# pollen-robotics/reachy2_symbolic_ik

Hardware: AMD Instinct MI355X
Metric: IK solves/sec (7-DoF r_arm, batched poses) (higher is better)
Workload: dtype f64; 1 GPU; config2: r_arm is_reachable + theta_to_joints_func(interval[0]), 1048576 random reachable poses per GPU; poses_per_gpu=1048576, theta_policy=interval[0], collective=none

## Files before the change

reachy2_symbolic_ik_amd/csrc/rsik_device.hpp:

```cpp
#pragma once

#include <hip/hip_runtime.h>
#include <stdint.h>

#include "../../include/rsik.h"
#include "rsik_math.hpp"

namespace rsik {

#ifdef RSIK_HOT_ONLY
#define RSIK_RARE(c) (false)
#else
#define RSIK_RARE(c) (__builtin_expect(!!(c), 0))
#endif


#ifdef RSIK_ISA_MARKS
#define RSIK_MARK(name) asm volatile("; RSIK_MARK " name)
#else
#define RSIK_MARK(name)
#endif

constexpr double kPi = 3.141592653589793;
constexpr double kTwoPi = 2 * kPi;
// ... 150 lines not shown
    else if (fabs(mid - kPi) <= 1e-7) { first = -2 * half_diff; third = 0.0; }
    else { first = half_sum - half_diff; third = half_sum + half_diff; }
    mid -= kPi / 2;
    eul[0] = first; eul[1] = mid; eul[2] = third;
#pragma unroll
    for (int k = 0; k < 3; k++) {
        if (eul[k] < -kPi) eul[k] += kTwoPi;
        else if (eul[k] > kPi) eul[k] -= kTwoPi;
    }
}

struct Frame {
    V3 c0, c1, c2;
};
__device__ __forceinline__ bool frame_is_special(V3 u) {
    if (!RSIK_RARE(fmax(fabs(u.y), fabs(u.z)) < 2e-8)) return false;
    return np_isclose(0.0, u.y) && np_isclose(0.0, u.z);
}
__device__ __forceinline__ V3 frame_c0(V3 u) {
    V3 c0 = u;
    if (RSIK_RARE(frame_is_special(u))) {
        if (np_isclose(1.0, u.x)) c0 = {1, 0, 0};
        else if (np_isclose(1.0, -u.x)) c0 = {-1, 0, 0};
    }
    return c0;
}
__device__ __forceinline__ Frame frame_from_unit(V3 u, double h) {
    Frame F;
    double yh = u.y * h, zh = u.z * h;
    double yzh = u.y * zh;
    F.c0 = u;
    F.c1 = {-u.y, fma(-u.y, yh, 1.0), -yzh};
    F.c2 = {-u.z, -yzh, fma(-u.z, zh, 1.0)};
    if (RSIK_RARE(frame_is_special(u))) {
        if (np_isclose(1.0, u.x)) { F.c0 = {1, 0, 0}; F.c1 = {0, 1, 0}; F.c2 = {0, 0, 1}; }
        else if (np_isclose(1.0, -u.x)) { F.c0 = {-1, 0, 0}; F.c1 = {0, 1, 0}; F.c2 = {0, 0, -1}; }
    }
    return F;
}
__device__ __forceinline__ Frame frame_from_unit(V3 u) { return frame_from_unit(u, fast_rcp(1.0 + u.x)); }

struct Reach {
    int state;
    bool ok;
    double i0, i1;
    double ct0, st0;
    double ct1, st1;
    V3 pos;
    V3 w;
    V3 c2;
    double r2;
    V3 n2;
    V3 a1, a2;
    int stage;
};

template <class Acc>
__device__ __forceinline__ V3 cvec(const Acc& A, int off) {
    return {A(off), A(off + 1), A(off + 2)};
}

struct Goal {
    V3 woff, toff, xg;
    V3 tw;
};
template <class Acc>
__device__ __forceinline__ Goal make_goal(const Acc& A, const Rot& Rg) {
    const V3 tl = cvec(A, RSIK_C_TIPL);
    Goal g;
    g.woff = {Rg.m[0] * tl.x + Rg.m[1] * tl.y + Rg.m[2] * tl.z, Rg.m[3] * tl.x + Rg.m[4] * tl.y + Rg.m[5] * tl.z,
              Rg.m[6] * tl.x + Rg.m[7] * tl.y + Rg.m[8] * tl.z};
    g.toff = {fma(Rg.m[0], tl.x, Rg.m[1] * tl.y), fma(Rg.m[3], tl.x, Rg.m[4] * tl.y), fma(Rg.m[6], tl.x, Rg.m[7] * tl.y)};
    g.xg = Rg.col0();
    g.tw = {-(Rg.m[2] * tl.z), -(Rg.m[5] * tl.z), -(Rg.m[8] * tl.z)};
    return g;
}
template <class Acc>
__device__ __forceinline__ Goal goal_from_euler_tipz(const Acc& A, double roll, double pitch, double yaw) {
    const double ang[3] = {roll, pitch, yaw};
    double sn[3], cs[3];
    fast_sincos_n<3>(ang, sn, cs);
    const double sa = sn[0], ca = cs[0], sb = sn[1], cb = cs[1], sc = sn[2], cc = cs[2];
    const double tz = A(RSIK_C_TIPL + 2);
    Goal g;
    g.woff = {fma(cc * sb, ca, sc * sa) * tz, fma(sc * sb, ca, -(cc * sa)) * tz, (cb * ca) * tz};
    g.toff = {0.0, 0.0, 0.0};
    g.xg = {cc * cb, sc * cb, -sb};
    g.tw = {-g.woff.x, -g.woff.y, -g.woff.z};
    return g;
}
__device__ __forceinline__ V3 wrist_position(const V3& woff, V3 pos) { return woff + pos; }

template <bool V>
struct BoolC {
    __device__ __forceinline__ constexpr operator bool() const { return V; }
};
template <bool KEEP, bool GEOM_ONLY, class NL, class Acc>
__device__ Reach reach_impl(const Acc& A, V3 pos_in, const V3 woff, const NL no_limits_v) {
    const bool NO_LIMITS = no_limits_v;
    Reach r;
    r.ok = false;
    r.i0 = r.i1 = __builtin_nan("");
    const V3 s = cvec(A, RSIK_C_SHOULDER);
    const double u = A(RSIK_C_UPPER_ARM), f = A(RSIK_C_FOREARM);
    const double bl = A(RSIK_C_BACKWARD), pm = A(RSIK_C_PROJ_MARGIN), upf = A(RSIK_C_UPF);

    V3 gp = pos_in;
    V3 dv = gp - s;
    const double ss0 = dot_d(dv, dv);
    int st = RSIK_STATE_REACHABLE;
    if (RSIK_RARE(ss0 > A(RSIK_C_MAX_LEN_SQ))) {
        double nd = sqrt_cr(ss0) + pm;
        gp = madd(dv * fast_rcp(nd), A(RSIK_C_MAX_LEN), s);
        st = RSIK_STATE_POSE_OUT_OF_REACH;
    }
    if (RSIK_RARE(gp.x < bl)) {
        gp.x = bl;
        st = RSIK_STATE_BACKWARD_POSE;
    }
    r.state = st;
    r.stage = 0;
    if (KEEP) { r.pos = gp; r.w = gp; r.c2 = gp; r.n2 = gp; r.a1 = gp; r.a2 = gp; r.r2 = 0.0; r.ct0 = 1.0; r.st0 = 0.0; r.ct1 = 1.0; r.st1 = 0.0; }
    if (!NO_LIMITS && st != RSIK_STATE_REACHABLE) return r;
    r.stage = 1;

    RSIK_MARK("reach_wrist");
    V3 w = wrist_position(woff, gp);
    if (RSIK_RARE(w.x < bl)) {
        double diff = bl - w.x;
        gp.x = gp.x + diff;
        if (NO_LIMITS) w = wrist_position(woff, gp);
        else w.x = w.x + diff;
    }
    V3 P = w - s;
    double dsw, inv_d;
    sqrt_rsqrt(dot_d(P, P), dsw, inv_d);
    double d = dsw;
    V3 self_pos = gp;
    if (NO_LIMITS) {
        if (RSIK_RARE(dsw > upf)) {
            double nd = fabs(dsw) + pm;
            V3 nw = madd((w - s) * fast_rcp(nd), upf, s);
            self_pos = gp + (nw - w);
            w = nw;
            P = w - s;
            sqrt_rsqrt(dot_d(P, P), d, inv_d);
        }
    } else {
        if (RSIK_RARE(dsw > upf)) {
            r.state = RSIK_STATE_WRIST_OUT_OF_RANGE;
            if (KEEP) { r.pos = gp; r.w = w; }
            return r;
        }
    }
    if (RSIK_RARE(dsw < A(RSIK_C_MIN_DIST))) {
        const double t = fabs(dsw) + pm;
        const double k = A(RSIK_C_MIN_DIST) * fast_rcp(t);
        const double km1 = k - 1.0;
        gp = madd(P, km1, gp);
        w = madd(P, km1, w);
        self_pos = gp;
        P = P * k;
        d = dsw * k;
        inv_d = inv_d * (t * A(RSIK_C_INV_MIN_DIST));
    }

    RSIK_MARK("reach_circle");
    if (RSIK_RARE(d > upf)) {
        r.state = RSIK_STATE_SHOULD_NOT_HAPPEN;
        if (KEEP) { r.pos = self_pos; r.w = w; }
        return r;
    }
    r.pos = self_pos;
    r.w = w;
    V3 n2 = P * inv_d;
    double r2, ir2;
    double kk;
    double fh;
    V3 c2;
    {
        double d2 = d * d, k = d2 - f * f + u * u;
        double rad = 4 * d2 * (u * u) - k * k;
        const double m = d + P.x;
        const double g = rad * (m * m);
        double irad, srad;
        if (RSIK_RARE(!(g > 0.0))) {
            irad = (rad != 0.0) ? rsqrt_fast(rad) : 0.0;
            srad = rad * irad;
            fh = fast_rcp(1.0 + n2.x);
        } else {
            const double z = rsqrt_fast(g);
            irad = z * m;
            srad = rad * irad;
            fh = d * (z * srad);
        }
        const double hid = 0.5 * inv_d;
        r2 = hid * srad;
        ir2 = (d + d) * irad;
        kk = k * hid;
        c2 = s + n2 * kk;
    }
    RSIK_MARK("reach_frame");
    Frame F2 = frame_from_unit(n2, fh);
    r.c2 = c2; r.r2 = r2; r.n2 = n2; r.a1 = F2.c1; r.a2 = F2.c2;
    r.stage = 2;
    if (NO_LIMITS || GEOM_ONLY) {
        r.ok = true; r.state = RSIK_STATE_REACHABLE; r.i0 = -kPi; r.i1 = kPi;
        r.ct0 = -1.0; r.st0 = -1.2246467991473532e-16;
        r.ct1 = -1.0; r.st1 = 1.2246467991473532e-16;
        return r;
    }

    RSIK_MARK("reach_limit_side");
    V3 N1 = woff * A(RSIK_C_INV_GRIP);
    double r1 = A(RSIK_C_WRIST_R);

    V3 p1 = N1 * A(RSIK_C_WRIST_AX), p2 = c2 - w;
    const V3 f1 = frame_c0(N1);
    const double tlx = -dot_d(f1, p1);
    const double side_val = dot_d(f1, p2) + tlx;
    bool side_ok = side_val > 0;
    r.state = side_ok ? RSIK_STATE_REACHABLE : RSIK_STATE_LIMITED_BY_WRIST;
    r.ok = side_ok;
    auto whole_or_nothing = [&]() {
        r.i0 = side_ok ? -kPi : __builtin_nan("");
        r.i1 = side_ok ? kPi : __builtin_nan("");
        r.ct0 = -1.0; r.st0 = -1.2246467991473532e-16;
        r.ct1 = -1.0; r.st1 = 1.2246467991473532e-16;
    };

    RSIK_MARK("reach_line");
    const V3 N2 = n2;
    {
        const double Ap = dot(N1, F2.c1), Bp = dot(N1, F2.c2);
        const double R2 = fma(Ap, Ap, Bp * Bp);
        const double Dp = -side_val * ir2;
        const double disc = fma(-Dp, Dp, R2);
        const double n2b = (kk - d) - A(RSIK_C_WRIST_AX) * dot(N1, N2);
        const bool exact = (ir2 == 0.0) || (R2 < 1e-12) || (fabs(disc) < 1e-8) ||
                           (fabs(side_val - n2b) <= 2e-8 + 2e-5 * fabs(n2b));
        if (!RSIK_RARE(exact)) {
            if (disc < 0) { whole_or_nothing(); return r; }
            r.ok = true;
            r.state = RSIK_STATE_REACHABLE;
            const double rd = R2 * disc;
            const double z = rsqrt_fast(R2 * rd);
            const double sal = disc * z;
            const double cal = Dp * (rd * (z * z));
            const double c0 = fma(Ap, cal, Bp * sal), s0 = fma(Bp, cal, -(Ap * sal));
            const double c1 = fma(Ap, cal, -(Bp * sal)), s1 = fma(Bp, cal, Ap * sal);
            const double ss[2] = {s0, s1}, cc[2] = {c0, c1};
            double aa[2];
            unit_atan2_n<2>(A.utab, ss, cc, aa);
            r.i0 = aa[0]; r.i1 = aa[1];
            r.ct0 = c0; r.st0 = s0;
            r.ct1 = c1; r.st1 = s1;
            return r;
        }
    }
    const double mg = A(RSIK_C_NORMAL_MARGIN);
    V3 cr = cross(N1, N2);
    const double crcr = dot(cr, cr);
    if (RSIK_RARE(crcr < 4.0 * (mg * mg) + 1e-30)) {
        bool par = (fabs(N2.x - N1.x) < mg && fabs(N2.y - N1.y) < mg && fabs(N2.z - N1.z) < mg) ||
                   (fabs(N2.x + N1.x) < mg && fabs(N2.y + N1.y) < mg && fabs(N2.z + N1.z) < mg);
        if (par) { whole_or_nothing(); return r; }
    }
    const double inv_nv = rsqrt_fast(crcr);
    V3 v = cr * inv_nv;
    V3 v1 = cross(v, N1);
    V3 b = p2 - p1;
    double t0 = dot(N2, b) * inv_nv;
    double t1 = dot(N1, b) * inv_nv;
    if (RSIK_RARE(np_isclose(t1, t0))) { whole_or_nothing(); return r; }
    V3 q = madd(v1, t0, p1);

    RSIK_MARK("reach_circle_line");
    V3 a1 = F2.c1, a2 = F2.c2;
    const double r1sq = r1 * r1;
    const double disc4 = fma(-t0, t0, r1sq);
    double ly1, lz1, ly2, lz2;
    double by, bz;
    if (RSIK_RARE(fabs(disc4) < 1e-9 * r1sq)) {
        V3 wv = q - p1;
        const double qa = v.x * v.x + v.y * v.y + v.z * v.z;
        const double qb = 2 * (v.x * wv.x + v.y * wv.y + v.z * wv.z);
        const double qc = (wv.x * wv.x + wv.y * wv.y + wv.z * wv.z) - r1 * r1;
        const double disc = qb * qb - 4 * qa * qc;
        if (disc < 0) { whole_or_nothing(); return r; }
        const double oy = -dot(a1, p2), oz = -dot(a2, p2);
        r.ok = true;
        r.state = RSIK_STATE_REACHABLE;
        const double inv_2qa = fma(-0.5, qa, 1.0);
        if (disc == 0) {
            double t = -qb * inv_2qa;
            V3 p = madd(v, t, q);
            double ly = dot(a1, p) + oy, lz = dot(a2, p) + oz;
            double ang = fast_atan2(lz, ly);
            double il = rsqrt_fast(ly * ly + lz * lz);
            r.i0 = ang; r.i1 = ang; r.ct0 = ly * il; r.st0 = lz * il; r.ct1 = r.ct0; r.st1 = r.st0;
            return r;
        }
        double sq = sqrt_cr(disc);
        double ta = (-qb + sq) * inv_2qa, tb = (-qb - sq) * inv_2qa;
        V3 pa = madd(v, ta, q), pb = madd(v, tb, q);
        ly1 = (dot(a1, pa) + oy) * ir2; lz1 = (dot(a2, pa) + oz) * ir2;
        ly2 = (dot(a1, pb) + oy) * ir2; lz2 = (dot(a2, pb) + oz) * ir2;
        by = 0.5 * (ly1 + ly2); bz = 0.5 * (lz1 + lz2);
    } else {
        if (disc4 < 0) { whole_or_nothing(); return r; }
        r.ok = true;
        r.state = RSIK_STATE_REACHABLE;
        const double hr = (disc4 * rsqrt_fast(disc4)) * ir2;
        const V3 dq = q - p2;
        by = dot(a1, dq) * ir2; bz = dot(a2, dq) * ir2;
        const double vy = dot(a1, v) * hr, vz = dot(a2, v) * hr;
        ly1 = by + vy; lz1 = bz + vz;
        ly2 = by - vy; lz2 = bz - vz;
    }
    RSIK_MARK("reach_atan2x2");
    double ang1, ang2;
    {
        const double ss[2] = {lz1, lz2}, cc[2] = {ly1, ly2};
        double aa[2];
        unit_atan2_n<2>(A.utab, ss, cc, aa);
        ang1 = aa[0]; ang2 = aa[1];
    }
    RSIK_MARK("reach_mid_select");
    double sm, cm;
    const double bb = fma(by, by, bz * bz);
    if (RSIK_RARE(bb < 1e-12)) {
        fast_sincos((ang1 + ang2) / 2, &sm, &cm);
    } else {
        double ib = rsqrt_fast(bb);
        ib = (fabs(ang1 - ang2) > kPi) ? -ib : ib;
        cm = by * ib; sm = bz * ib;
    }
    const double fa1 = dot(f1, a1), fa2 = dot(f1, a2);
    const bool inside = fma(r2, fma(cm, fa1, sm * fa2), side_val) > 0;
    const bool first = inside != (ang2 < ang1);
    r.i0 = first ? ang1 : ang2;
    r.i1 = first ? ang2 : ang1;
    r.ct0 = first ? ly1 : ly2;
    r.st0 = first ? lz1 : lz2;
    r.ct1 = first ? ly2 : ly1;
    r.st1 = first ? lz2 : lz1;
    return r;
}

template <bool NO_LIMITS, bool KEEP = true, class Acc>
__device__ __forceinline__ Reach reach_g(const Acc& A, V3 pos_in, const V3 woff) {
    return reach_impl<KEEP, false>(A, pos_in, woff, BoolC<NO_LIMITS>{});
}

template <bool NO_LIMITS, bool KEEP = true, class Acc>
__device__ __forceinline__ Reach reach(const Acc& A, V3 pos_in, const Rot& Rg) {
    return reach_g<NO_LIMITS, KEEP>(A, pos_in, make_goal(A, Rg).woff);
}

__device__ __forceinline__ V3 elbow_on_circle(const Reach& r, double ct, double st) {
    double y = r.r2 * ct, z = r.r2 * st;
    return madd(r.a1, y, madd(r.a2, z, r.c2));
}

template <bool EXACT = true, class Acc>
__device__ __forceinline__ bool above_singularity_plane(const Acc& A, V3 e) {
    if constexpr (EXACT) return e.z > (e.x - A(RSIK_C_ES)) * A(RSIK_C_SING_COEFF) + A(RSIK_C_ES + 2) - A(RSIK_C_SING_OFFSET);
    else return e.z > fma(e.x, A(RSIK_C_SING_COEFF), A(RSIK_C_PLANE_K));
}
template <bool PLANE = true, class Acc>
__device__ __forceinline__ bool is_elbow_ok(const Acc& A, V3 e) {
    bool ok = e.y * A(RSIK_C_SIDE) < -0.2;
    if constexpr (PLANE) ok = ok && (e.z < (e.x - A(RSIK_C_ES)) * A(RSIK_C_SING_COEFF) + A(RSIK_C_ES + 2) - A(RSIK_C_SING_OFFSET));
    return ok;
}

struct JointsOut {
    double j[7];
    V3 elbow;
    bool projected;
    bool sing;
    double c4, s4, c5, s5, c6, s6;
};

typedef const __attribute__((address_space(1))) double* GConst;
template <bool FRESH, bool TIPZ = false, class Acc, class Prev = const double*>
__device__ JointsOut joints_from_theta_g(const Acc& A, Reach& r, const Goal& G, double ct, double st, Prev prev) {
    RSIK_MARK("joints_elbow");
    JointsOut o;
    V3 e = elbow_on_circle(r, ct, st);
    o.projected = false;
    if (RSIK_RARE(above_singularity_plane<!FRESH>(A, e))) {
        const V3 v3 = cvec(A, RSIK_C_PLANE_N), pc = cvec(A, RSIK_C_PROJ_CENTER);
        const V3 d1 = e - pc;
        const V3 V = madd(v3, -dot(d1, v3), d1);
        const V3 ne = madd(V, A(RSIK_C_PROJ_RADIUS) * rsqrt_fast(dot(V, V)), pc);
        const V3 shift = ne - e;
        e = ne;
        if constexpr (FRESH) {
            r.w = r.w + shift;
        } else {
            r.pos = r.pos + shift;
            r.w = wrist_position(G.woff, r.pos);
        }
        o.projected = true;
    }
    RSIK_MARK("joints_shoulder");
    o.elbow = e;
    const double u = A(RSIK_C_UPPER_ARM), f = A(RSIK_C_FOREARM);
    auto to_shoulder = [&](V3 p) -> V3 {
        return {fma(A(RSIK_C_MST + 0), p.x, fma(A(RSIK_C_MST + 1), p.y, fma(A(RSIK_C_MST + 2), p.z, A(RSIK_C_TSH + 0)))),
                fma(A(RSIK_C_MST + 3), p.x, fma(A(RSIK_C_MST + 4), p.y, fma(A(RSIK_C_MST + 5), p.z, A(RSIK_C_TSH + 1)))),
                fma(A(RSIK_C_MST + 6), p.x, fma(A(RSIK_C_MST + 7), p.y, fma(A(RSIK_C_MST + 8), p.z, A(RSIK_C_TSH + 2))))};
    };
    V3 q = to_shoulder(e);
    double cphi, sphi, rho;
    const bool sing_sp = RSIK_RARE(q.x == 0 && q.z == 0);
    if (sing_sp) {
        double s_, c_;
        fast_sincos(prev[0], &s_, &c_);
        cphi = c_; sphi = -s_; rho = 0.0;
    } else {
        const double rho2 = fma(q.x, q.x, q.z * q.z);
        const double irho = rsqrt_fast(rho2);
        rho = rho2 * irho;
        cphi = q.x * irho; sphi = q.z * irho;
    }
    const double iL = A(RSIK_C_INV_U);
    double cr = rho * iL, srs = q.y * iL;
    V3 g0 = {cr * cphi, srs, cr * sphi};
    V3 g1 = {-srs * cphi, cr, -srs * sphi};
    V3 g2 = {-sphi, 0.0, cphi};
    auto rot_g = [&](V3 a) -> V3 { return {dot(g0, a), dot(g1, a), fma(g2.x, a.x, g2.z * a.z)}; };
    auto to_elbow = [&](V3 p) -> V3 {
        V3 a = rot_g(to_shoulder(p));
        a.x -= u;
        return a;
    };
    RSIK_MARK("joints_elbow_angles");
    V3 pw = to_elbow(r.w);
    double sigma, ca, sa;
    const bool sing_ey = RSIK_RARE(pw.y == 0 && pw.z == 0);
    if (sing_ey) {
// ... 484 lines not shown
```

reachy2_symbolic_ik_amd/csrc/rsik_kernel_nearest.hpp:

```cpp
#pragma once

namespace rsik {

struct NearestArgs {
    int64_t n;
    const double* in[6];
    const uint8_t* arm;
    int theta_policy;
    int n_theta;
    int theta_per_pose;
    int skip_projected;
    const double* theta_in;
    union {
        double prev[7];
        const double* prev_rows;
    };
    const double* seed;
    double weights[7];
    int32_t* index;
    double* theta;
    double* joints;
    double* elbow;
    double* cost;
    uint8_t* projected;
// ... 25 lines not shown
                                                const double* __restrict__ lds_rows) {
    __builtin_amdgcn_s_waitcnt(0xC07F);
    __builtin_amdgcn_wave_barrier();
    const int total = nrows * W;
    double* dst = out + wave_base * W;
#pragma unroll
    for (int k = 0; k < W; k++) {
        if (k * 64 < PW * W) {
            const int idx = k * 64 + lane;
            if (idx < total) st_stream(dst + idx, lds_rows[idx]);
        }
    }
    __builtin_amdgcn_wave_barrier();
}

#ifndef RSIK_NEAREST_MIN_WAVES
#define RSIK_NEAREST_MIN_WAVES 1
#endif
template <int MIXED, bool TIPZ, bool PREV_ROWS, int L>
__global__ __launch_bounds__(kBlock, RSIK_NEAREST_MIN_WAVES) void solve_nearest_kernel(const NearestArgs K) {
    static_assert(L == 1 || L == 8 || L == 64, "lanes per pose");
    constexpr int PW = 64 / L;
    constexpr int PB = kBlock / L;
    __shared__ SharedTables lds_tab;
    __shared__ double lds[kBlock / 64][64 * 10];
    const int lane = threadIdx.x & 63;
    const int wave = __builtin_amdgcn_readfirstlane(threadIdx.x >> 6);
    const int64_t tile0 = (int64_t)blockIdx.x * PB;
    const int64_t left = K.n - tile0;
    const unsigned rows = left < PB ? (unsigned)left : (unsigned)PB;
    const unsigned sub = (unsigned)lane & (L - 1);
    const unsigned pw = (unsigned)lane / L;
    const unsigned t = (unsigned)wave * PW + pw;
    const unsigned tt = (t < rows ? t : rows - 1) & (PB - 1);
    const bool lead = sub == 0;
    const bool live = t < rows && lead;

    double in[6];
#pragma unroll
    for (int k = 0; k < 6; k++) in[k] = ld_stream(K.in[k] + tile0 + tt);
    warm_and_stage_tables<MIXED>(K, lds_tab);
    const AccNearest<MIXED> A = kernarg_acc<AccNearest<MIXED>, NearestArgs>(lds_tab, (MIXED != 0 && K.arm[tile0 + tt] != 0) ? 1 : 0);
    double* lds_wave = lds[wave];

    const bool invalid = !all_finite(in);
    const V3 pos = {in[0], in[1], in[2]};
    Goal G;
    if constexpr (TIPZ) {
        G = goal_from_euler_tipz(A, in[3], in[4], in[5]);
    } else {
        const Rot Rg = rot_from_euler(in[3], in[4], in[5]);
        G = make_goal(A, Rg);
    }
    Reach r = reach_g<false, false>(A, pos, G.woff);
    if (RSIK_RARE(invalid)) reach_invalid_input(r);
    store_reach(K, live, tile0, t, r);
    if (rows <= (unsigned)(wave * PW)) return;

    const int wave_rows = rows - wave * PW < PW ? (int)(rows - wave * PW) : PW;
    const int64_t wave_base = tile0 + wave * PW;
    {
        const double* src = K.seed + wave_base * 7;
#pragma unroll
        for (int k = 0; k < 7; k++) {
            if (k * 64 < PW * 7) {
                const int idx = k * 64 + lane;
                if (idx < wave_rows * 7) lds_wave[idx] = ld_stream(src + idx);
            }
        }
        __builtin_amdgcn_s_waitcnt(0xC07F);
        __builtin_amdgcn_wave_barrier();
    }
    const double* seed = lds_wave + (tt - wave * PW) * 7;
    double* jrow = lds_wave + pw * 7;
    double* erow = lds_wave + 64 * 7 + pw * 3;

    const bool want_elbow = K.elbow != nullptr;
    const bool fraction = K.theta_policy != RSIK_THETA_EXPLICIT;
    const bool per_pose = K.theta_per_pose != 0;
    const bool skip_projected = K.skip_projected != 0;
    const double fa = r.i0;
    double fb = r.i1;
    if (fa > fb) fb += kTwoPi;
    const double fspan = fb - fa;
    const V3 wrist = r.w;
    const double* th_col = K.theta_in + tile0 + tt;

    double best_c = __builtin_inf();
    int best_k = kNoSample;
    double win_theta = __builtin_nan("");
    bool win_projected = false, won = false;
    const int rounds = (K.n_theta + L - 1) / L;
#pragma clang loop unroll(disable)
    for (int it = 0; it <= rounds; it++) {
        const bool last = it == rounds;
        if (last) {
            if constexpr (L > 1) nearest_of_group<L>(best_c, best_k);
        }
        const int k = last ? best_k : it * L + (int)sub;
        if (r.ok && k < K.n_theta) {
            const double th_in = per_pose ? th_col[(int64_t)k * K.n] : K.theta_in[k];
            double theta = th_in;
            if (fraction) theta = fa + th_in * fspan;
            double ct, st;
            fast_sincos(theta, &st, &ct);
            r.w = wrist;
            JointsOut o;
            if constexpr (PREV_ROWS) o = joints_from_theta_g<true, TIPZ>(A, r, G, ct, st, (GConst)(K.prev_rows + (tile0 + tt) * 7));
            else o = joints_from_theta_g<true, TIPZ>(A, r, G, ct, st, (const double*)K.prev);
            if (!last) {
                double c = 0.0;
#pragma unroll
                for (int q = 0; q < 7; q++) {
                    const double d = angle_diff(o.j[q], seed[q]);
                    c = c + (K.weights[q] * d) * d;
                }
                if (!(skip_projected && o.projected) && nearer(c, k, best_c, best_k)) { best_c = c; best_k = k; }
            } else {
                won = true;
                win_theta = theta;
                win_projected = o.projected;
                if (lead) {
#pragma unroll
                    for (int q = 0; q < 7; q++) jrow[q] = o.j[q];
                    if (want_elbow) { erow[0] = o.elbow.x; erow[1] = o.elbow.y; erow[2] = o.elbow.z; }
                }
            }
        }
        branch_stores_stay();
    }
    if (!won && lead) {
        const double nan = opaque(__builtin_nan(""));
#pragma unroll
        for (int q = 0; q < 7; q++) jrow[q] = nan;
        if (want_elbow) { erow[0] = nan; erow[1] = nan; erow[2] = nan; }
        branch_stores_stay();
    }
    if (L == 1 && wave_rows == 64) {
        if (K.joints) flush_rows_full<7>(K.joints, wave_base, lane, lds_wave);
        if (want_elbow) flush_rows_full<3>(K.elbow, wave_base, lane, lds_wave + 64 * 7);
    } else {
        if (K.joints) flush_pose_rows<7, PW>(K.joints, wave_base, wave_rows, lane, lds_wave);
        if (want_elbow) flush_pose_rows<3, PW>(K.elbow, wave_base, wave_rows, lane, lds_wave + 64 * 7);
    }
    if (live) {
        if (K.index) st_stream(K.index + tile0 + t, (int32_t)(won ? best_k : -1));
        if (K.theta) st_stream(K.theta + tile0 + t, win_theta);
        if (K.cost) st_stream(K.cost + tile0 + t, won ? sqrt(best_c) : __builtin_nan(""));
        if (K.projected) st_stream(K.projected + tile0 + t, (uint8_t)(win_projected ? 1 : 0));
    }
}

}
```

reachy2_symbolic_ik_amd/csrc/rsik_kernel_path.hpp:

```cpp
#pragma once

namespace rsik {

struct PathArgs {
    int64_t n;
    int64_t n_steps;
    const double* in[6];
    const uint8_t* arm;
    int theta_policy;
    int n_theta;
    int theta_per_pose;
    int skip_projected;
    int unwind;
    const double* theta_in;
    double prev[7];
    const double* start;
    double weights[7];
    uint8_t* back;
    int32_t* index;
    double* theta;
    double* joints;
    double* elbow;
    uint8_t* projected;
    double* step_cost;
// ... 111 lines not shown
    bool have_uprev = has_start;
    const int trips = (T + 63) >> 6;
#pragma clang loop unroll(disable)
    for (int it = 0; it < T + trips; it++) {
        const bool out = it >= T;
        if (it == T) {
            double end_a = last_a;
            int end_k = (pmask >> lane) & 1 ? lane : kNoSample;
            nearest_of_group<64>(end_a, end_k);
            if (lane == 0) {
                if (K.cost) st_stream(K.cost + path, solved ? end_a : __builtin_nan(""));
                if (K.n_solved) st_stream(K.n_solved + path, (int32_t)solved);
            }
            int cur = __builtin_amdgcn_readfirstlane(end_k);
            unsigned mine = kPathNone;
            for (int tb = T - 1; tb >= 0; tb -= 8) {
                unsigned b[8];
#pragma unroll
                for (int u = 0; u < 8; u++) {
                    const int t = tb - u;
                    b[u] = (t >= 0 && lane < NT) ? (unsigned)back[(int64_t)t * NT + lane] : kPathNone;
                }
#pragma unroll
                for (int u = 0; u < 8; u++) {
                    const int t = tb - u;
                    if (t >= 0) {
                        const bool was_solved = __builtin_amdgcn_ballot_w64(b[u] != kPathNone) != 0;
                        if ((t & 63) == lane) mine = was_solved ? (unsigned)cur : kPathNone;
                        if (was_solved) cur = __builtin_amdgcn_readlane((int)b[u], cur & 63);
                        if ((t & 63) == 0 && t + lane < T) winners[t + lane] = (uint8_t)mine;
                    }
                }
            }
        }
        const int wp_raw = out ? ((it - T) << 6) + lane : it;
        const bool live = wp_raw < T;
        const int wp = live ? wp_raw : T - 1;
        int k = lane;
        if (out) k = live ? (int)winners[wp] : (int)kPathNone;
        const int64_t row = (int64_t)wp * n + path;

        double in[6];
#pragma unroll
        for (int c = 0; c < 6; c++) in[c] = ld_stream(K.in[c] + row);
        const bool invalid = !all_finite(in);
        const V3 pos = {in[0], in[1], in[2]};
        Goal G;
        if constexpr (TIPZ) {
            G = goal_from_euler_tipz(A, in[3], in[4], in[5]);
        } else {
            const Rot Rg = rot_from_euler(in[3], in[4], in[5]);
            G = make_goal(A, Rg);
        }
        Reach r = reach_g<false, false>(A, pos, G.woff);
        if (RSIK_RARE(invalid)) reach_invalid_input(r);
        if (out) store_reach(K, live, row, 0u, r);

        const bool run = r.ok && k < NT && !lost;
        JointsOut o;
        double theta = __builtin_nan("");
        bool cand = false;
        if (run) {
            const double th_in = per_pose ? K.theta_in[(int64_t)k * T * n + row] : K.theta_in[k];
            theta = th_in;
            if (fraction) {
                const double fa = r.i0;
                double fb = r.i1;
                if (fa > fb) fb += kTwoPi;
                theta = fa + th_in * (fb - fa);
            }
            double ct, st;
            fast_sincos(theta, &st, &ct);
            o = joints_from_theta_g<true, TIPZ>(A, r, G, ct, st, (const double*)K.prev);
            cand = !(skip_projected && o.projected);
#pragma unroll
            for (int q = 0; q < 7; q++) cand = cand && o.j[q] == o.j[q];
        }

        if (!out) {
            const unsigned long long cmask = __builtin_amdgcn_ballot_w64(cand);
            unsigned bp = kPathNone;
            if (cmask != 0) {
                double* cur_rows = lds_wave + cs * (64 * kPathRow);
                const double* prev_rows = lds_wave + (cs ^ 1) * (64 * kPathRow);
                double a = __builtin_inf();
                if (cand) {
                    double* mine = cur_rows + lane * kPathRow;
#pragma unroll
                    for (int q = 0; q < 7; q++) mine[q] = o.j[q];
                    if (solved == 0) {
                        a = has_start ? path_cost_at(w, o.j, carry) : 0.0;
                        bp = kPathFirst;
                    } else {
                        unsigned long long m = pmask;
                        int i = __builtin_ctzll(m);
                        m &= m - 1;
                        PathRow pr = path_row(prev_rows + i * kPathRow);
                        for (;;) {
                            const bool more = m != 0;
                            const int i_next = more ? __builtin_ctzll(m) : i;
                            m &= m - 1;
                            const PathRow pr_next = path_row(prev_rows + i_next * kPathRow);
                            const double v = pr.v[3].y + path_cost(w, o.j, pr);
                            if (v < a) { a = v; bp = (unsigned)i; }
                            if (!more) break;
                            pr = pr_next;
                            i = i_next;
                        }
                    }
                    mine[7] = a;
                }
                last_a = a;
                pmask = cmask;
                cs ^= 1;
                solved++;
                path_lds_fence();
            }
            if (lane < NT) back[(int64_t)it * NT + lane] = (uint8_t)bp;
        } else {
            double* jrow = lds_wave + lane * 7;
            double* erow = lds_wave + 64 * 7 + lane * 3;
            const int t0 = (it - T) << 6;
            const bool won = run && live;
            bool win_projected = false;
            if (won) {
#pragma unroll
// ... 71 lines not shown
```

reachy2_symbolic_ik_amd/csrc/rsik_kernel_solve.hpp:

```cpp
#pragma once

namespace rsik {

#ifndef RSIK_BLOCK
#define RSIK_BLOCK 256
#endif
constexpr int kBlock = RSIK_BLOCK;

struct SolveArgs {
    int64_t n;
    const double* in[6];
    const uint8_t* arm;
    int theta_policy;
    const double* theta_in;
    union {
        double prev[7];
        const double* prev_rows;
    };
    double* joints;
    double* interval;
    double* elbow;
    uint8_t* reachable;
    uint8_t* state;
    ArmC arms[2];
// ... 201 lines not shown
        const f64x2 iv = {r.i0, r.i1};
        st_stream(reinterpret_cast<f64x2*>(K.interval + 2 * tile0) + t, iv);
    }
    if (K.reachable) st_stream(K.reachable + tile0 + t, (uint8_t)(r.ok ? 1 : 0));
    if (K.state) st_stream(K.state + tile0 + t, (uint8_t)r.state);
}

template <int MIXED, bool TIPZ, bool PREV_ROWS = false>
__global__ __launch_bounds__(kBlock, RSIK_SOLVE_MIN_WAVES) void solve_kernel(const SolveArgs K) {
    __shared__ SharedTables lds_tab;
    __shared__ double lds[kBlock / 64][64 * 10];
    const int lane = threadIdx.x & 63;
    const int wave = __builtin_amdgcn_readfirstlane(threadIdx.x >> 6);
    const int64_t tile0 = (int64_t)blockIdx.x * kBlock;
    const int64_t left = K.n - tile0;
    const unsigned rows = left < kBlock ? (unsigned)left : (unsigned)kBlock;
    const unsigned t = threadIdx.x & (kBlock - 1);
    const unsigned tt = (t < rows ? t : rows - 1) & (kBlock - 1);
    const bool live = t < rows;

#ifdef RSIK_CLOCK_PROBE
    const uint64_t probe_c0 = __builtin_readcyclecounter(), probe_r0 = __builtin_amdgcn_s_memrealtime();
#endif
#ifdef RSIK_TIMELINE_PROBE
    const uint64_t probe_t0 = __builtin_amdgcn_s_memrealtime();
#endif
    double in[6];
#pragma unroll
    for (int k = 0; k < 6; k++) in[k] = ld_stream(K.in[k] + tile0 + tt);
    warm_and_stage_tables<MIXED>(K, lds_tab);
#ifdef RSIK_TIMELINE_PROBE
    const uint64_t probe_t1 = __builtin_amdgcn_s_memrealtime();
    uint64_t probe_mid = 0, probe_goal = 0, probe_reach = 0;
#define RSIK_SOLVE_PROBE(v) do { __builtin_amdgcn_sched_barrier(0); v = __builtin_amdgcn_s_memrealtime(); __builtin_amdgcn_sched_barrier(0); } while (0)
#else
#define RSIK_SOLVE_PROBE(v) do { } while (0)
#endif
    const AccK<MIXED> A = kernarg_acc<AccK<MIXED>, SolveArgs>(lds_tab, (MIXED != 0 && K.arm[tile0 + tt] != 0) ? 1 : 0);
    double* lds_wave = lds[wave];

    const bool invalid = !all_finite(in);
    const V3 pos = {in[0], in[1], in[2]};
    Goal G;
    if constexpr (TIPZ) {
        G = goal_from_euler_tipz(A, in[3], in[4], in[5]);
    } else {
        RSIK_MARK("euler");
        const Rot Rg = rot_from_euler(in[3], in[4], in[5]);
        RSIK_MARK("goal");
        G = make_goal(A, Rg);
    }
    RSIK_MARK("reach_start");
    RSIK_SOLVE_PROBE(probe_goal);
    Reach r = reach_g<false, false>(A, pos, G.woff);
    RSIK_SOLVE_PROBE(probe_reach);
    if (RSIK_RARE(invalid)) reach_invalid_input(r);
    RSIK_MARK("after_reach");

    const bool want_elbow = K.elbow != nullptr;
    if (K.theta_policy != RSIK_THETA_NONE) {
        double* jrow = lds_wave + lane * 7;
        double* erow = lds_wave + 64 * 7 + lane * 3;
        if (r.ok) {
            double ct = r.ct0, st = r.st0;
            if (K.theta_policy != RSIK_THETA_INTERVAL0) {
                const double th_in = K.theta_in[tile0 + tt];
                double theta = th_in;
                if (K.theta_policy != RSIK_THETA_EXPLICIT) {
                    double a = r.i0, b = r.i1;
                    if (a > b) b += kTwoPi;
                    theta = a + th_in * (b - a);
                }
                fast_sincos(theta, &st, &ct);
            }
            if constexpr (PREV_ROWS) {
                JointsOut o = joints_from_theta_g<true, TIPZ>(A, r, G, ct, st, (GConst)(K.prev_rows + (tile0 + tt) * 7));
                RSIK_MARK("stores");
#pragma unroll
                for (int k = 0; k < 7; k++) jrow[k] = o.j[k];
                if (want_elbow) { erow[0] = o.elbow.x; erow[1] = o.elbow.y; erow[2] = o.elbow.z; }
                branch_stores_stay();
            } else {
                JointsOut o = joints_from_theta_g<true, TIPZ>(A, r, G, ct, st, (const double*)K.prev);
                RSIK_MARK("stores");
#pragma unroll
                for (int k = 0; k < 7; k++) jrow[k] = o.j[k];
                if (want_elbow) { erow[0] = o.elbow.x; erow[1] = o.elbow.y; erow[2] = o.elbow.z; }
                branch_stores_stay();
            }
        } else {
            const double nan = opaque(__builtin_nan(""));
#pragma unroll
            for (int k = 0; k < 7; k++) jrow[k] = nan;
            if (want_elbow) { erow[0] = nan; erow[1] = nan; erow[2] = nan; }
            branch_stores_stay();
        }
#ifdef RSIK_TIMELINE_PROBE
        probe_mid = __builtin_amdgcn_s_memrealtime();
#endif
        const int64_t wave_base = tile0 + wave * 64;
        if (rows >= (unsigned)(wave * 64 + 64)) {
            if (K.joints) flush_rows_full<7>(K.joints, wave_base, lane, lds_wave);
            if (want_elbow) flush_rows_full<3>(K.elbow, wave_base, lane, lds_wave + 64 * 7);
        } else if (rows > (unsigned)(wave * 64)) {
            if (K.joints) flush_rows<7>(K.joints, wave_base, K.n, lane, lds_wave);
            if (want_elbow) flush_rows<3>(K.elbow, wave_base, K.n, lane, lds_wave + 64 * 7);
        }
    }
    store_reach(K, live, tile0, t, r);
#ifdef RSIK_TIMELINE_PROBE
    if (lane < 4 && K.interval && live) {
        __builtin_amdgcn_s_waitcnt(0);
        const uint64_t t3 = __builtin_amdgcn_s_memrealtime();
        const uint32_t hw = __builtin_amdgcn_s_getreg((4 << 0) | (0 << 6) | (31 << 11));
        const uint32_t xcc = __builtin_amdgcn_s_getreg((20 << 0) | (0 << 6) | (31 << 11));
        double2 iv;
        if (lane == 0) iv = {(double)probe_t0, (double)probe_t1};
        else if (lane == 1) iv = {(double)probe_mid, (double)t3};
        else if (lane == 2) iv = {(double)hw, (double)xcc};
        else iv = {(double)probe_goal, (double)probe_reach};
        reinterpret_cast<double2*>(K.interval)[tile0 + t] = iv;
    }
#endif
#ifdef RSIK_CLOCK_PROBE
    if (lane == 0 && K.interval && live) {
        const uint64_t c1 = __builtin_readcyclecounter(), r1 = __builtin_amdgcn_s_memrealtime();
        double2 iv = {(double)(c1 - probe_c0), (double)(r1 - probe_r0)};
        reinterpret_cast<double2*>(K.interval)[tile0 + t] = iv;
    }
#endif
}

__device__ __forceinline__ void goal_from_m12(const double (&m)[12], Rot& Rg, V3& pos, int mode, bool* special = nullptr) {
#pragma unroll
    for (int k = 0; k < 9; k++) Rg.m[k] = m[k];
    if (special) {
// ... 54 lines not shown
```

reachy2_symbolic_ik_amd/csrc/rsik_kernel_sweep.hpp:

```cpp
#pragma once

namespace rsik {

struct SweepArgs {
    int64_t n;
    const double* in[6];
    const uint8_t* arm;
    int theta_policy;
    int n_theta;
    int theta_per_pose;
    const double* theta_in;
    union {
        double prev[7];
        const double* prev_rows;
    };
    double* joints;
    double* elbow;
    uint8_t* projected;
    double* theta;
    double* interval;
    uint8_t* reachable;
    uint8_t* state;
    ArmC arms[2];
};

template <int MIXED>
struct AccSweep : AccK<MIXED> {};

#ifndef RSIK_SWEEP_MIN_WAVES
#define RSIK_SWEEP_MIN_WAVES 1
#endif
template <int MIXED, bool TIPZ, bool PREV_ROWS>
__global__ __launch_bounds__(kBlock, RSIK_SWEEP_MIN_WAVES) void solve_sweep_kernel(const SweepArgs K) {
    __shared__ SharedTables lds_tab;
    __shared__ double lds[kBlock / 64][64 * 10];
    const int lane = threadIdx.x & 63;
    const int wave = __builtin_amdgcn_readfirstlane(threadIdx.x >> 6);
    const int64_t tile0 = (int64_t)blockIdx.x * kBlock;
    const int64_t left = K.n - tile0;
    const unsigned rows = left < kBlock ? (unsigned)left : (unsigned)kBlock;
    const unsigned t = threadIdx.x & (kBlock - 1);
    const unsigned tt = (t < rows ? t : rows - 1) & (kBlock - 1);
    const bool live = t < rows;

    double in[6];
#pragma unroll
    for (int k = 0; k < 6; k++) in[k] = ld_stream(K.in[k] + tile0 + tt);
    warm_and_stage_tables<MIXED>(K, lds_tab);
    const AccSweep<MIXED> A = kernarg_acc<AccSweep<MIXED>, SweepArgs>(lds_tab, (MIXED != 0 && K.arm[tile0 + tt] != 0) ? 1 : 0);
    double* lds_wave = lds[wave];

    const bool invalid = !all_finite(in);
    const V3 pos = {in[0], in[1], in[2]};
    Goal G;
    if constexpr (TIPZ) {
        G = goal_from_euler_tipz(A, in[3], in[4], in[5]);
    } else {
        const Rot Rg = rot_from_euler(in[3], in[4], in[5]);
        G = make_goal(A, Rg);
    }
    Reach r = reach_g<false, false>(A, pos, G.woff);
    if (RSIK_RARE(invalid)) reach_invalid_input(r);
    store_reach(K, live, tile0, t, r);
    if (rows <= (unsigned)(wave * 64)) return;

    const bool want_elbow = K.elbow != nullptr;
    const bool full = rows >= (unsigned)(wave * 64 + 64);
    const bool fraction = K.theta_policy != RSIK_THETA_EXPLICIT;
    const bool per_pose = K.theta_per_pose != 0;
    const int64_t wave_base = tile0 + wave * 64;
    double* jrow = lds_wave + lane * 7;
    double* erow = lds_wave + 64 * 7 + lane * 3;
    const double fa = r.i0;
    double fb = r.i1;
    if (fa > fb) fb += kTwoPi;
    const double fspan = fb - fa;
    const V3 wrist = r.w;
    if (!r.ok) {
        const double nan = opaque(__builtin_nan(""));
#pragma unroll
        for (int k = 0; k < 7; k++) jrow[k] = nan;
        erow[0] = nan; erow[1] = nan; erow[2] = nan;
        branch_stores_stay();
    }
    const __attribute__((address_space(4))) double* grid = (const __attribute__((address_space(4))) double*)K.theta_in;
    const double* th_col = K.theta_in + tile0 + tt;
    double* jout = K.joints;
    double* eout = K.elbow;
    uint8_t* pout = K.projected ? K.projected + tile0 + t : nullptr;
    double* tout = K.theta ? K.theta + tile0 + t : nullptr;
#pragma clang loop unroll(disable)
    for (int k = 0; k < K.n_theta; k++) {
        const double th_in = per_pose ? *th_col : grid[k];
        double theta = th_in;
        if (fraction) theta = fa + th_in * fspan;
        bool projected = false;
        if (r.ok) {
            double ct, st;
            fast_sincos(theta, &st, &ct);
            r.w = wrist;
            if constexpr (PREV_ROWS) {
                JointsOut o = joints_from_theta_g<true, TIPZ>(A, r, G, ct, st, (GConst)(K.prev_rows + (tile0 + tt) * 7));
#pragma unroll
                for (int q = 0; q < 7; q++) jrow[q] = o.j[q];
                if (want_elbow) { erow[0] = o.elbow.x; erow[1] = o.elbow.y; erow[2] = o.elbow.z; }
                projected = o.projected;
                branch_stores_stay();
            } else {
                JointsOut o = joints_from_theta_g<true, TIPZ>(A, r, G, ct, st, (const double*)K.prev);
#pragma unroll
                for (int q = 0; q < 7; q++) jrow[q] = o.j[q];
                if (want_elbow) { erow[0] = o.elbow.x; erow[1] = o.elbow.y; erow[2] = o.elbow.z; }
                projected = o.projected;
                branch_stores_stay();
            }
        } else {
            theta = __builtin_nan("");
        }
        if (full) {
            flush_rows_full<7>(jout, wave_base, lane, lds_wave);
            if (want_elbow) flush_rows_full<3>(eout, wave_base, lane, lds_wave + 64 * 7);
        } else {
            flush_rows<7>(jout, wave_base, K.n, lane, lds_wave);
            if (want_elbow) flush_rows<3>(eout, wave_base, K.n, lane, lds_wave + 64 * 7);
        }
        if (live) {
            if (pout) st_stream(pout, (uint8_t)(projected ? 1 : 0));
            if (tout) st_stream(tout, theta);
        }
        jout += K.n * 7;
        if (want_elbow) eout += K.n * 3;
        if (pout) pout += K.n;
        if (tout) tout += K.n;
        th_col += K.n;
    }
}

}
```

Baseline: 35.35 billion solves/s.

## Skip explicit elbow-circle frame; compute axes implicitly from normal and h

Adds an AXES=false path in which reach no longer builds the full orthonormal frame for the elbow circle. It stores only the normal, the frame factor h and an axial flag, and elbow_on_circle rebuilds the circle point from these. The wrist-side test and the line projection coefficients are rewritten algebraically from dot products of N1 and n2, and the reference frame computation runs only on rare paths. This reduces live state and FLOPs in the hot kernels (solve, sweep, path, nearest), at the cost of extra special-case branches and a changed exactness test (r2 threshold instead of ir2==0) that could alter results near the edge cases.

```diff
diff --git a/reachy2_symbolic_ik_amd/csrc/rsik_device.hpp b/reachy2_symbolic_ik_amd/csrc/rsik_device.hpp
--- a/reachy2_symbolic_ik_amd/csrc/rsik_device.hpp
+++ b/reachy2_symbolic_ik_amd/csrc/rsik_device.hpp
@@ -226,6 +226,8 @@
     double r2;
     V3 n2;
     V3 a1, a2;
+    double h;
+    bool axial;
     int stage;
 };
 
@@ -269,7 +271,7 @@
 struct BoolC {
     __device__ __forceinline__ constexpr operator bool() const { return V; }
 };
-template <bool KEEP, bool GEOM_ONLY, class NL, class Acc>
+template <bool KEEP, bool GEOM_ONLY, bool AXES = true, class NL, class Acc>
 __device__ Reach reach_impl(const Acc& A, V3 pos_in, const V3 woff, const NL no_limits_v) {
     const bool NO_LIMITS = no_limits_v;
     Reach r;
@@ -294,7 +296,7 @@
     }
     r.state = st;
     r.stage = 0;
-    if (KEEP) { r.pos = gp; r.w = gp; r.c2 = gp; r.n2 = gp; r.a1 = gp; r.a2 = gp; r.r2 = 0.0; r.ct0 = 1.0; r.st0 = 0.0; r.ct1 = 1.0; r.st1 = 0.0; }
+    if (KEEP) { r.pos = gp; r.w = gp; r.c2 = gp; r.n2 = gp; r.a1 = gp; r.a2 = gp; r.h = 0.0; r.axial = false; r.r2 = 0.0; r.ct0 = 1.0; r.st0 = 0.0; r.ct1 = 1.0; r.st1 = 0.0; }
     if (!NO_LIMITS && st != RSIK_STATE_REACHABLE) return r;
     r.stage = 1;
 
@@ -375,8 +377,10 @@
         c2 = s + n2 * kk;
     }
     RSIK_MARK("reach_frame");
-    Frame F2 = frame_from_unit(n2, fh);
-    r.c2 = c2; r.r2 = r2; r.n2 = n2; r.a1 = F2.c1; r.a2 = F2.c2;
+    const bool axial = frame_is_special(n2);
+    Frame F2;
+    if constexpr (AXES) { F2 = frame_from_unit(n2, fh); r.a1 = F2.c1; r.a2 = F2.c2; }
+    r.c2 = c2; r.r2 = r2; r.n2 = n2; r.h = fh; r.axial = axial;
     r.stage = 2;
     if (NO_LIMITS || GEOM_ONLY) {
         r.ok = true; r.state = RSIK_STATE_REACHABLE; r.i0 = -kPi; r.i1 = kPi;
@@ -389,14 +393,22 @@
     V3 N1 = woff * A(RSIK_C_INV_GRIP);
     double r1 = A(RSIK_C_WRIST_R);
 
-    V3 p1 = N1 * A(RSIK_C_WRIST_AX), p2 = c2 - w;
-    const V3 f1 = frame_c0(N1);
-    const double tlx = -dot_d(f1, p1);
-    const double side_val = dot_d(f1, p2) + tlx;
-    bool side_ok = side_val > 0;
-    r.state = side_ok ? RSIK_STATE_REACHABLE : RSIK_STATE_LIMITED_BY_WRIST;
-    r.ok = side_ok;
+    V3 p1, p2, f1;
+    auto side_reference = [&]() -> double {
+        p1 = N1 * A(RSIK_C_WRIST_AX); p2 = c2 - w; f1 = frame_c0(N1);
+        const double tlx = -dot_d(f1, p1);
+        return dot_d(f1, p2) + tlx;
+    };
+    const double nyz = fma(N1.y, n2.y, N1.z * n2.z);
+    const double n1n2 = fma(N1.x, n2.x, nyz);
+    const double kd = kk - d;
+    double side_val = fma(kd, n1n2, -A(RSIK_C_WRIST_AX));
+    double side_dec = side_val;
+    if (RSIK_RARE(frame_is_special(N1))) side_dec = side_reference();
     auto whole_or_nothing = [&]() {
+        const bool side_ok = side_dec > 0;
+        r.state = side_ok ? RSIK_STATE_REACHABLE : RSIK_STATE_LIMITED_BY_WRIST;
+        r.ok = side_ok;
         r.i0 = side_ok ? -kPi : __builtin_nan("");
         r.i1 = side_ok ? kPi : __builtin_nan("");
         r.ct0 = -1.0; r.st0 = -1.2246467991473532e-16;
@@ -406,12 +418,17 @@
     RSIK_MARK("reach_line");
     const V3 N2 = n2;
     {
-        const double Ap = dot(N1, F2.c1), Bp = dot(N1, F2.c2);
+        const double T = fma(fh, nyz, N1.x);
+        double Ap = fma(-n2.y, T, N1.y), Bp = fma(-n2.z, T, N1.z);
+        if (RSIK_RARE(axial)) {
+            const Frame Fs = frame_from_unit(n2, fh);
+            Ap = dot(N1, Fs.c1); Bp = dot(N1, Fs.c2);
+        }
         const double R2 = fma(Ap, Ap, Bp * Bp);
         const double Dp = -side_val * ir2;
         const double disc = fma(-Dp, Dp, R2);
-        const double n2b = (kk - d) - A(RSIK_C_WRIST_AX) * dot(N1, N2);
-        const bool exact = (ir2 == 0.0) || (R2 < 1e-12) || (fabs(disc) < 1e-8) ||
+        const double n2b = kd - A(RSIK_C_WRIST_AX) * n1n2;
+        const bool exact = !(r2 > 1e-3) || (R2 < 1e-12) || (fabs(disc) < 1e-8) ||
                            (fabs(side_val - n2b) <= 2e-8 + 2e-5 * fabs(n2b));
         if (!RSIK_RARE(exact)) {
             if (disc < 0) { whole_or_nothing(); return r; }
@@ -432,6 +449,12 @@
             return r;
         }
     }
+    side_val = side_dec = side_reference();
+    if constexpr (!AXES) {
+        F2 = frame_from_unit(n2, fh);
+        if (!KEEP) { r.n2.y = -F2.c1.x; r.n2.z = -F2.c2.x; }
+    }
+    const double fa1 = dot(f1, F2.c1), fa2 = dot(f1, F2.c2);
     const double mg = A(RSIK_C_NORMAL_MARGIN);
     V3 cr = cross(N1, N2);
     const double crcr = dot(cr, cr);
@@ -510,7 +533,6 @@
         ib = (fabs(ang1 - ang2) > kPi) ? -ib : ib;
         cm = by * ib; sm = bz * ib;
     }
-    const double fa1 = dot(f1, a1), fa2 = dot(f1, a2);
     const bool inside = fma(r2, fma(cm, fa1, sm * fa2), side_val) > 0;
     const bool first = inside != (ang2 < ang1);
     r.i0 = first ? ang1 : ang2;
@@ -522,9 +544,9 @@
     return r;
 }
 
-template <bool NO_LIMITS, bool KEEP = true, class Acc>
+template <bool NO_LIMITS, bool KEEP = true, bool AXES = true, class Acc>
 __device__ __forceinline__ Reach reach_g(const Acc& A, V3 pos_in, const V3 woff) {
-    return reach_impl<KEEP, false>(A, pos_in, woff, BoolC<NO_LIMITS>{});
+    return reach_impl<KEEP, false, AXES>(A, pos_in, woff, BoolC<NO_LIMITS>{});
 }
 
 template <bool NO_LIMITS, bool KEEP = true, class Acc>
@@ -532,9 +554,20 @@
     return reach_g<NO_LIMITS, KEEP>(A, pos_in, make_goal(A, Rg).woff);
 }
 
+template <bool AXES = true>
 __device__ __forceinline__ V3 elbow_on_circle(const Reach& r, double ct, double st) {
-    double y = r.r2 * ct, z = r.r2 * st;
-    return madd(r.a1, y, madd(r.a2, z, r.c2));
+    if constexpr (AXES) {
+        const double y = r.r2 * ct, z = r.r2 * st;
+        return madd(r.a1, y, madd(r.a2, z, r.c2));
+    }
+    if (RSIK_RARE(r.axial)) {
+        const double y = r.r2 * ct, z = r.r2 * st;
+        return {r.c2.x, y + r.c2.y, r.n2.x > 0 ? r.c2.z + z : r.c2.z - z};
+    }
+    const double S = fma(r.n2.y, ct, r.n2.z * st);
+    const double Sh = S * r.h;
+    const V3 c = {-S, fma(-Sh, r.n2.y, ct), fma(-Sh, r.n2.z, st)};
+    return madd(c, r.r2, r.c2);
 }
 
 template <bool EXACT = true, class Acc>
@@ -558,11 +591,11 @@
 };
 
 typedef const __attribute__((address_space(1))) double* GConst;
-template <bool FRESH, bool TIPZ = false, class Acc, class Prev = const double*>
+template <bool FRESH, bool TIPZ = false, bool AXES = true, class Acc, class Prev = const double*>
 __device__ JointsOut joints_from_theta_g(const Acc& A, Reach& r, const Goal& G, double ct, double st, Prev prev) {
     RSIK_MARK("joints_elbow");
     JointsOut o;
-    V3 e = elbow_on_circle(r, ct, st);
+    V3 e = elbow_on_circle<AXES>(r, ct, st);
     o.projected = false;
     if (RSIK_RARE(above_singularity_plane<!FRESH>(A, e))) {
         const V3 v3 = cvec(A, RSIK_C_PLANE_N), pc = cvec(A, RSIK_C_PROJ_CENTER);
diff --git a/reachy2_symbolic_ik_amd/csrc/rsik_kernel_nearest.hpp b/reachy2_symbolic_ik_amd/csrc/rsik_kernel_nearest.hpp
--- a/reachy2_symbolic_ik_amd/csrc/rsik_kernel_nearest.hpp
+++ b/reachy2_symbolic_ik_amd/csrc/rsik_kernel_nearest.hpp
@@ -101,7 +101,7 @@
         const Rot Rg = rot_from_euler(in[3], in[4], in[5]);
         G = make_goal(A, Rg);
     }
-    Reach r = reach_g<false, false>(A, pos, G.woff);
+    Reach r = reach_g<false, false, false>(A, pos, G.woff);
     if (RSIK_RARE(invalid)) reach_invalid_input(r);
     store_reach(K, live, tile0, t, r);
     if (rows <= (unsigned)(wave * PW)) return;
@@ -155,8 +155,8 @@
             fast_sincos(theta, &st, &ct);
             r.w = wrist;
             JointsOut o;
-            if constexpr (PREV_ROWS) o = joints_from_theta_g<true, TIPZ>(A, r, G, ct, st, (GConst)(K.prev_rows + (tile0 + tt) * 7));
-            else o = joints_from_theta_g<true, TIPZ>(A, r, G, ct, st, (const double*)K.prev);
+            if constexpr (PREV_ROWS) o = joints_from_theta_g<true, TIPZ, false>(A, r, G, ct, st, (GConst)(K.prev_rows + (tile0 + tt) * 7));
+            else o = joints_from_theta_g<true, TIPZ, false>(A, r, G, ct, st, (const double*)K.prev);
             if (!last) {
                 double c = 0.0;
 #pragma unroll
diff --git a/reachy2_symbolic_ik_amd/csrc/rsik_kernel_path.hpp b/reachy2_symbolic_ik_amd/csrc/rsik_kernel_path.hpp
--- a/reachy2_symbolic_ik_amd/csrc/rsik_kernel_path.hpp
+++ b/reachy2_symbolic_ik_amd/csrc/rsik_kernel_path.hpp
@@ -187,7 +187,7 @@
             const Rot Rg = rot_from_euler(in[3], in[4], in[5]);
             G = make_goal(A, Rg);
         }
-        Reach r = reach_g<false, false>(A, pos, G.woff);
+        Reach r = reach_g<false, false, false>(A, pos, G.woff);
         if (RSIK_RARE(invalid)) reach_invalid_input(r);
         if (out) store_reach(K, live, row, 0u, r);
 
@@ -206,7 +206,7 @@
             }
             double ct, st;
             fast_sincos(theta, &st, &ct);
-            o = joints_from_theta_g<true, TIPZ>(A, r, G, ct, st, (const double*)K.prev);
+            o = joints_from_theta_g<true, TIPZ, false>(A, r, G, ct, st, (const double*)K.prev);
             cand = !(skip_projected && o.projected);
 #pragma unroll
             for (int q = 0; q < 7; q++) cand = cand && o.j[q] == o.j[q];
diff --git a/reachy2_symbolic_ik_amd/csrc/rsik_kernel_solve.hpp b/reachy2_symbolic_ik_amd/csrc/rsik_kernel_solve.hpp
--- a/reachy2_symbolic_ik_amd/csrc/rsik_kernel_solve.hpp
+++ b/reachy2_symbolic_ik_amd/csrc/rsik_kernel_solve.hpp
@@ -277,7 +277,7 @@
     }
     RSIK_MARK("reach_start");
     RSIK_SOLVE_PROBE(probe_goal);
-    Reach r = reach_g<false, false>(A, pos, G.woff);
+    Reach r = reach_g<false, false, false>(A, pos, G.woff);
     RSIK_SOLVE_PROBE(probe_reach);
     if (RSIK_RARE(invalid)) reach_invalid_input(r);
     RSIK_MARK("after_reach");
@@ -299,14 +299,14 @@
                 fast_sincos(theta, &st, &ct);
             }
             if constexpr (PREV_ROWS) {
-                JointsOut o = joints_from_theta_g<true, TIPZ>(A, r, G, ct, st, (GConst)(K.prev_rows + (tile0 + tt) * 7));
+                JointsOut o = joints_from_theta_g<true, TIPZ, false>(A, r, G, ct, st, (GConst)(K.prev_rows + (tile0 + tt) * 7));
                 RSIK_MARK("stores");
 #pragma unroll
                 for (int k = 0; k < 7; k++) jrow[k] = o.j[k];
                 if (want_elbow) { erow[0] = o.elbow.x; erow[1] = o.elbow.y; erow[2] = o.elbow.z; }
                 branch_stores_stay();
             } else {
-                JointsOut o = joints_from_theta_g<true, TIPZ>(A, r, G, ct, st, (const double*)K.prev);
+                JointsOut o = joints_from_theta_g<true, TIPZ, false>(A, r, G, ct, st, (const double*)K.prev);
                 RSIK_MARK("stores");
 #pragma unroll
                 for (int k = 0; k < 7; k++) jrow[k] = o.j[k];
diff --git a/reachy2_symbolic_ik_amd/csrc/rsik_kernel_sweep.hpp b/reachy2_symbolic_ik_amd/csrc/rsik_kernel_sweep.hpp
--- a/reachy2_symbolic_ik_amd/csrc/rsik_kernel_sweep.hpp
+++ b/reachy2_symbolic_ik_amd/csrc/rsik_kernel_sweep.hpp
@@ -59,7 +59,7 @@
         const Rot Rg = rot_from_euler(in[3], in[4], in[5]);
         G = make_goal(A, Rg);
     }
-    Reach r = reach_g<false, false>(A, pos, G.woff);
+    Reach r = reach_g<false, false, false>(A, pos, G.woff);
     if (RSIK_RARE(invalid)) reach_invalid_input(r);
     store_reach(K, live, tile0, t, r);
     if (rows <= (unsigned)(wave * 64)) return;
@@ -100,14 +100,14 @@
             fast_sincos(theta, &st, &ct);
             r.w = wrist;
             if constexpr (PREV_ROWS) {
-                JointsOut o = joints_from_theta_g<true, TIPZ>(A, r, G, ct, st, (GConst)(K.prev_rows + (tile0 + tt) * 7));
+                JointsOut o = joints_from_theta_g<true, TIPZ, false>(A, r, G, ct, st, (GConst)(K.prev_rows + (tile0 + tt) * 7));
 #pragma unroll
                 for (int q = 0; q < 7; q++) jrow[q] = o.j[q];
                 if (want_elbow) { erow[0] = o.elbow.x; erow[1] = o.elbow.y; erow[2] = o.elbow.z; }
                 projected = o.projected;
                 branch_stores_stay();
             } else {
-                JointsOut o = joints_from_theta_g<true, TIPZ>(A, r, G, ct, st, (const double*)K.prev);
+                JointsOut o = joints_from_theta_g<true, TIPZ, false>(A, r, G, ct, st, (const double*)K.prev);
 #pragma unroll
                 for (int q = 0; q < 7; q++) jrow[q] = o.j[q];
                 if (want_elbow) { erow[0] = o.elbow.x; erow[1] = o.elbow.y; erow[2] = o.elbow.z; }
```

Result: no change. 35.25 billion solves/s, median of 2 (-0.3%).
